# EryiXie/PlaneRecNet

Measured on AMD Instinct MI355X. Metric: img/s fwd+bwd @480×640 ResNet101-DCN, 1/2/4/8 MI355X + roofline %, higher is better.
Workload: dtype f32 (tensors and accumulation fp32; plain GEMMs and the tap-walked 4x4/s2, 1x1/s2 and sub-pixel convolutions >= 300 tiles: 2xfp16-piece split MFMA, fp32 accumulate; fp32-only rate in fp32_only_run)

## Files before the change

### planerecnet_amd/csrc/prn_wgrad16.hip

```cpp
#include "prn_common.h"

namespace {

typedef __attribute__((ext_vector_type(8))) _Float16 h8_t;
typedef __attribute__((ext_vector_type(2))) _Float16 h2_t;
typedef __attribute__((ext_vector_type(2))) float f2_t;
typedef __attribute__((ext_vector_type(16))) float f16x_t;

constexpr unsigned W16_OOB = 0x80000000u;
constexpr int W16_PLANE = 128 * 32;
constexpr int W16_BUF = 4 * W16_PLANE;

struct Wg16Args {
  const float* dy; const float* x; float* out;
  int M, C, HW, B;
  int N;
  int tilesM, tilesC, splits, chunks;
  long long zdy, zx;
  long long zout;
  int nz;
  int wide;
  int ngroup;
  const float* gx[PRN_WGRAD_GROUP_MAX];
  const float* gdy[PRN_WGRAD_GROUP_MAX];
};

__device__ __forceinline__ const float* w16_kernarg_ptr(size_t member_offset, int i) {
  typedef __attribute__((address_space(4))) const uint64_t* kptr;
  kptr base = (kptr)__builtin_amdgcn_kernarg_segment_ptr();
  return reinterpret_cast<const float*>(base[member_offset / 8 + i]);
}

__device__ __forceinline__ float quad_max(float v) {
  const int a = __builtin_amdgcn_mov_dpp(__float_as_int(v), 0xB1, 0xF, 0xF, true);
  v = fmaxf(v, __int_as_float(a));
  const int b = __builtin_amdgcn_mov_dpp(__float_as_int(v), 0x4E, 0xF, 0xF, true);
  return fmaxf(v, __int_as_float(b));
}

template <int NP>
__global__ __launch_bounds__(256) __attribute__((amdgpu_waves_per_eu(3, 3))) void wgrad16_kernel(const Wg16Args a) {
  __shared__ __attribute__((aligned(16))) unsigned char pieces[2 * W16_BUF];
  __shared__ int rowexp[2][256];
  __shared__ int scratch[4][64];
  const int t = threadIdx.x, lane = t & 63, wave = __builtin_amdgcn_readfirstlane(t >> 6);
  const int tiles = a.tilesM * a.tilesC;
  const int lid = prn_xcd_remap(blockIdx.x, tiles * a.splits * a.nz);
  const int tile = lid % tiles, rest = lid / tiles;
  const int tm = tile % a.tilesM, tc = tile / a.tilesM;
  const int sp = rest % a.splits, z = rest / a.splits;
  const int q0 = (int)((long long)a.chunks * sp / a.splits), q1 = (int)((long long)a.chunks * (sp + 1) / a.splits);
  const int HW = a.HW;
  const float* dyz = a.ngroup > 0 ? w16_kernarg_ptr(offsetof(Wg16Args, gdy), z) : a.dy + (long long)z * a.zdy;
  const float* xz = a.ngroup > 0 ? w16_kernarg_ptr(offsetof(Wg16Args, gx), z) : a.x + (long long)z * a.zx;
  const __amdgpu_buffer_rsrc_t ars = __builtin_amdgcn_make_buffer_rsrc(const_cast<float*>(dyz), 0, a.B * a.M * HW * 4, 0x00020000);
  const __amdgpu_buffer_rsrc_t brs = __builtin_amdgcn_make_buffer_rsrc(const_cast<float*>(xz), 0, a.B * a.C * HW * 4, 0x00020000);

  const int quarter = t & 3, rsub = t >> 2;
  unsigned rowoff[4];
  int erun[4];
  unsigned wroff[4];
#pragma unroll
  for (int k = 0; k < 4; ++k) {
    const int rl = rsub + 64 * (k & 1);
    const int row = (k < 2 ? tm : tc) * 128 + rl;
    const bool ok = row < (k < 2 ? a.M : a.C);
    rowoff[k] = ok ? (unsigned)(row * HW * 4) : W16_OOB;
    erun[k] = -200;
    wroff[k] = (unsigned)((k < 2 ? 0 : 2 * W16_PLANE) + rl * 32 + (((quarter >> 1) ^ ((rl >> 2) & 1)) * 16) + (quarter & 1) * 8);
  }
  const unsigned imgA = (unsigned)(a.M * HW * 4), imgB = (unsigned)(a.C * HW * 4);
  int cb, cp;
  {
    const long long n = (long long)q0 * 16 + quarter * 4;
    cb = (int)(n / HW); cp = (int)(n - (long long)cb * HW);
  }
  float4 ld0[4], ld1[4];
  auto load_chunk = [&](float4 (&ld)[4]) {
    const unsigned past = (unsigned)((a.B - 1 - cb) >> 31) << 31;
    const unsigned pa = ((unsigned)cb * imgA + (unsigned)cp * 4u) | past, pb = ((unsigned)cb * imgB + (unsigned)cp * 4u) | past;
#pragma unroll
    for (int k = 0; k < 4; ++k)
      ld[k] = __builtin_bit_cast(float4, __builtin_amdgcn_raw_buffer_load_b128(k < 2 ? ars : brs, (int)((k < 2 ? pa : pb) + (rowoff[k] & 0x7fffffffu)) | (int)(rowoff[k] & 0x80000000u), 0, 0));
    cp += 16;
    const int wrap = (HW - 1 - cp) >> 31;
    cp -= HW & wrap; cb -= wrap;
  };
  auto cut_chunk = [&](const float4 (&ld)[4], int buf) {
    unsigned char* pb = pieces + buf * W16_BUF;
#pragma unroll
    for (int k = 0; k < 4; ++k) {
      const float4 v = ld[k];
      const float mx = quad_max(fmaxf(fmaxf(fabsf(v.x), fabsf(v.y)), fmaxf(fabsf(v.z), fabsf(v.w))));
      int ec = mx > 0.f ? __builtin_amdgcn_frexp_expf(mx) : -200;
      ec = ec < -100 ? (mx > 0.f ? -100 : -200) : ec;
      if (ec > erun[k] + 3) erun[k] = ec;
      const float s = __builtin_amdgcn_ldexpf(1.0f, 11 - (erun[k] < -100 ? -100 : erun[k]));
      const f2_t s2 = {s, s};
      const f2_t x0 = f2_t{v.x, v.y} * s2, x1 = f2_t{v.z, v.w} * s2;
      const h2_t h0 = __builtin_convertvector(x0, h2_t), h1 = __builtin_convertvector(x1, h2_t);
      const f2_t r0 = x0 - __builtin_convertvector(h0, f2_t), r1 = x1 - __builtin_convertvector(h1, f2_t);
      const h2_t l0 = __builtin_convertvector(r0, h2_t), l1 = __builtin_convertvector(r1, h2_t);
      uint2 hh, ll;
      hh.x = __builtin_bit_cast(unsigned, h0); hh.y = __builtin_bit_cast(unsigned, h1);
      ll.x = __builtin_bit_cast(unsigned, l0); ll.y = __builtin_bit_cast(unsigned, l1);
      *reinterpret_cast<uint2*>(pb + wroff[k]) = hh;
      *reinterpret_cast<uint2*>(pb + wroff[k] + W16_PLANE) = ll;
      if (quarter == 0) rowexp[buf][rsub + 64 * k] = erun[k];
    }
  };

  const int wm = wave >> 1, wn = wave & 1, r = lane & 31, g = lane >> 5;
  f16x_t acc[2][2];
#pragma unroll
  for (int i = 0; i < 2; ++i)
#pragma unroll
    for (int j = 0; j < 2; ++j)
#pragma unroll
      for (int e = 0; e < 16; ++e) acc[i][j][e] = 0.f;
  int prevA = -200, prevB = -200;
  auto mma_chunk = [&](int buf) {
    const int newA = rowexp[buf][wm * 64 + lane], newB = rowexp[buf][128 + wn * 64 + lane];
    const int dA = prevA - newA, dB = prevB - newB;
    prevA = newA; prevB = newB;
    if (__builtin_amdgcn_ballot_w64((dA | dB) != 0) != 0ull) {
      scratch[wave][lane] = dA;
      __builtin_amdgcn_wave_barrier();
#pragma unroll
      for (int j = 0; j < 2; ++j) {
        const int db = __shfl(dB, j * 32 + r, 64);
#pragma unroll
        for (int i = 0; i < 2; ++i)
#pragma unroll
          for (int e = 0; e < 16; ++e) {
            const int da = scratch[wave][i * 32 + (e >> 2) * 8 + g * 4 + (e & 3)];
            acc[i][j][e] = __builtin_amdgcn_ldexpf(acc[i][j][e], da + db);
          }
      }
      __builtin_amdgcn_wave_barrier();
    }
    const unsigned char* pb = pieces + buf * W16_BUF;
    h8_t ah[2], al[2], bh[2], bl[2];
#pragma unroll
    for (int u = 0; u < 2; ++u) {
      const int ra = wm * 64 + u * 32 + r, rb = wn * 64 + u * 32 + r;
      const unsigned oa = (unsigned)(ra * 32 + ((g ^ ((ra >> 2) & 1)) * 16)), ob = (unsigned)(2 * W16_PLANE + rb * 32 + ((g ^ ((rb >> 2) & 1)) * 16));
      ah[u] = *reinterpret_cast<const h8_t*>(pb + oa); al[u] = *reinterpret_cast<const h8_t*>(pb + oa + W16_PLANE);
      bh[u] = *reinterpret_cast<const h8_t*>(pb + ob); bl[u] = *reinterpret_cast<const h8_t*>(pb + ob + W16_PLANE);
    }
#pragma unroll
    for (int i = 0; i < 2; ++i)
#pragma unroll
      for (int j = 0; j < 2; ++j) {
        f16x_t c = acc[i][j];
        if (NP >= 4) c = __builtin_amdgcn_mfma_f32_32x32x16_f16(al[i], bl[j], c, 0, 0, 0);
        c = __builtin_amdgcn_mfma_f32_32x32x16_f16(al[i], bh[j], c, 0, 0, 0);
        c = __builtin_amdgcn_mfma_f32_32x32x16_f16(ah[i], bl[j], c, 0, 0, 0);
        c = __builtin_amdgcn_mfma_f32_32x32x16_f16(ah[i], bh[j], c, 0, 0, 0);
        acc[i][j] = c;
      }
  };

  const int nq = q1 - q0;
  if (nq > 0) {
    load_chunk(ld0);
    load_chunk(ld1);
    cut_chunk(ld0, 0);
    load_chunk(ld0);
    __syncthreads();
    int i = 0;
    for (; i + 1 < nq; i += 2) {
      cut_chunk(ld1, 1);
      load_chunk(ld1);
      __builtin_amdgcn_sched_barrier(0);
      mma_chunk(0);
      __syncthreads();
      cut_chunk(ld0, 0);
      load_chunk(ld0);
      __builtin_amdgcn_sched_barrier(0);
      mma_chunk(1);
      __syncthreads();
    }
    if (i < nq) mma_chunk(0);
  }

  scratch[wave][lane] = prevA;
  __builtin_amdgcn_wave_barrier();
  float* ob = a.out + ((long long)sp * a.nz + z) * a.zout;
  if (a.wide) {
    __syncthreads();
    float* cw = reinterpret_cast<float*>(pieces) + wave * (32 * 36);
    const int crow = lane >> 3, ccol = (lane & 7) * 4;
#pragma unroll
    for (int j = 0; j < 2; ++j) {
      const int eb = __shfl(prevB, j * 32 + r, 64);
      const int col4 = tc * 128 + wn * 64 + j * 32 + ccol;
#pragma unroll
      for (int i = 0; i < 2; ++i) {
#pragma unroll
        for (int e = 0; e < 16; ++e) {
          const int ro = (e >> 2) * 8 + g * 4 + (e & 3);
          const int ea = scratch[wave][i * 32 + ro];
          cw[ro * 36 + r] = (ea <= -200 || eb <= -200) ? 0.f : __builtin_amdgcn_ldexpf(acc[i][j][e], ea + eb - 22);
        }
        __builtin_amdgcn_wave_barrier();
#pragma unroll
        for (int q = 0; q < 4; ++q) {
          const int rl = crow + 8 * q, row = tm * 128 + wm * 64 + i * 32 + rl;
          const float4 v = *reinterpret_cast<const float4*>(&cw[rl * 36 + ccol]);
          if (row < a.M && col4 < a.C) *reinterpret_cast<float4*>(ob + (long long)row * a.C + col4) = v;
        }
        __builtin_amdgcn_wave_barrier();
      }
    }
    return;
  }
#pragma unroll
  for (int j = 0; j < 2; ++j) {
    const int col = tc * 128 + wn * 64 + j * 32 + r;
    const int eb = __shfl(prevB, j * 32 + r, 64);
    if (col >= a.C) continue;
#pragma unroll
    for (int i = 0; i < 2; ++i)
#pragma unroll
      for (int e = 0; e < 16; ++e) {
        const int rl = i * 32 + (e >> 2) * 8 + g * 4 + (e & 3), row = tm * 128 + wm * 64 + rl;
        const int ea = scratch[wave][rl];
        if (row < a.M) ob[(long long)row * a.C + col] = (ea <= -200 || eb <= -200) ? 0.f : __builtin_amdgcn_ldexpf(acc[i][j][e], ea + eb - 22);
      }
  }
}

}

int prn_wgrad16_plan(int M, int C, int64_t N, int HW, int nz, const prn_gemm_opts* o) {
  if (o == nullptr || o->wgrad_split == PRN_SPLIT_OFF) return 0;
  if (M <= 0 || C <= 0 || N <= 0 || nz <= 0 || nz >= 65536 || (HW & 3) != 0 || HW < 16 || N % HW != 0) return 0;
  if ((int64_t)M * N >= (1LL << 29) || (int64_t)C * N >= (1LL << 29)) return 0;
  const int64_t tiles = (int64_t)cdiv(M, 128) * cdiv(C, 128) * nz;
  const int chunks = cdiv(N, 16);
  if (o->wgrad_split != PRN_SPLIT_ALWAYS) {
    if ((int64_t)cdiv(M, 128) * 128 * 4 > (int64_t)M * 5 || (int64_t)cdiv(C, 128) * 128 * 4 > (int64_t)C * 5) return 0;
    if (2.0 * M * C * (double)N * nz < 0.25e9 * (double)o->split_min_gflop) return 0;
  }
  const int target = o->wgrad_wgs > 0 ? o->wgrad_wgs : 768;
  int64_t s = tiles >= target ? 1 : target / tiles;
  const int smax = chunks / 8 > 0 ? chunks / 8 : 1;
  if (s > smax) s = smax;
  if (s > 256) s = 256;
  s = prn_quantise_splits(tiles, (int)s);
  return s < 1 ? 1 : (int)s;
}

int prn_wgrad16_launch(const float* dy, const float* x, const float* const* gdy, const float* const* gx, int ngroup, float* out, int M, int C, int B, int HW, int nz,
                       int64_t zdy, int64_t zx, int splits, const prn_gemm_opts* o, hipStream_t st) {
  PRN_REQUIRE(out && splits >= 1 && (ngroup > 0 ? (gdy && gx && ngroup <= PRN_WGRAD_GROUP_MAX) : (dy && x)), "prn_wgrad16: bad arguments");
  Wg16Args a;
  a.dy = dy; a.x = x; a.out = out; a.M = M; a.C = C; a.HW = HW; a.B = B; a.N = B * HW;
  a.tilesM = cdiv(M, 128); a.tilesC = cdiv(C, 128); a.splits = splits; a.chunks = cdiv((int64_t)B * HW, 16);
  a.zdy = zdy; a.zx = zx; a.zout = (long long)M * C; a.nz = ngroup > 0 ? ngroup : nz; a.ngroup = ngroup;
  for (int i = 0; i < PRN_WGRAD_GROUP_MAX; ++i) {
    a.gx[i] = ngroup > 0 ? gx[i < ngroup ? i : 0] : nullptr; a.gdy[i] = ngroup > 0 ? gdy[i < ngroup ? i : 0] : nullptr;
    if (ngroup > 0) {
      PRN_REQUIRE(a.gx[i] && a.gdy[i] && (reinterpret_cast<uintptr_t>(a.gx[i]) & 15) == 0 && (reinterpret_cast<uintptr_t>(a.gdy[i]) & 15) == 0, "prn_wgrad16: null / unaligned tensor in the group");
    }
  }
  a.wide = (C & 3) == 0 && (reinterpret_cast<uintptr_t>(out) & 15) == 0;
  const dim3 grid((unsigned)(a.tilesM * a.tilesC * splits * a.nz)), block(256);
  if (o && o->split_products >= 4) hipLaunchKernelGGL(wgrad16_kernel<4>, grid, block, 0, st, a);
  else hipLaunchKernelGGL(wgrad16_kernel<3>, grid, block, 0, st, a);
  PRN_CHECK_LAUNCH("prn_wgrad16");
  return 0;
}
```

Measured before the change: 194.9.

## Interleave fp16 split conversion of next chunk with MFMAs in wgrad16

Adds a CUT variant of the split-fp16 weight-gradient kernel, enabled by default. It scans the next chunk's row maxima up front using integer bit comparisons and a cached scale/threshold, so exponents are recomputed only when a row's magnitude grows. The hi/lo split conversion and LDS stores are cut into parts and placed between the MFMA instructions of the current chunk, so VALU conversion work overlaps matrix work instead of running serially before it. It also uses v_max3 and fma_mix inline asm. The cost is higher register pressure, more sched_barrier constraints, and some risk that the read-before-write ordering on the alternate LDS buffer is wrong.

```diff
diff --git a/planerecnet_amd/csrc/prn_wgrad16.hip b/planerecnet_amd/csrc/prn_wgrad16.hip
--- a/planerecnet_amd/csrc/prn_wgrad16.hip
+++ b/planerecnet_amd/csrc/prn_wgrad16.hip
@@ -38,7 +38,21 @@
   return fmaxf(v, __int_as_float(b));
 }
 
-template <int NP>
+__device__ __forceinline__ unsigned quad_max_bits(unsigned v) {
+  const unsigned a = (unsigned)__builtin_amdgcn_update_dpp(0, (int)v, 0xB1, 0xF, 0xF, true);
+  v = v > a ? v : a;
+  const unsigned b = (unsigned)__builtin_amdgcn_update_dpp(0, (int)v, 0x4E, 0xF, 0xF, true);
+  return v > b ? v : b;
+}
+
+__device__ __forceinline__ unsigned absmax4_bits(const float4 v) {
+  float m;
+  asm("v_max3_f32 %0, |%1|, |%2|, |%3|" : "=v"(m) : "v"(v.x), "v"(v.y), "v"(v.z));
+  const unsigned mb = __float_as_uint(m), wb = __float_as_uint(v.w) & 0x7fffffffu;
+  return mb > wb ? mb : wb;
+}
+
+template <int NP, int CUT>
 __global__ __launch_bounds__(256) __attribute__((amdgpu_waves_per_eu(3, 3))) void wgrad16_kernel(const Wg16Args a) {
   __shared__ __attribute__((aligned(16))) unsigned char pieces[2 * W16_BUF];
   __shared__ int rowexp[2][256];
@@ -59,6 +73,8 @@
   const int quarter = t & 3, rsub = t >> 2;
   unsigned rowoff[4];
   int erun[4];
+  float scl[4];
+  int thr[4];
   unsigned wroff[4];
 #pragma unroll
   for (int k = 0; k < 4; ++k) {
@@ -66,7 +82,7 @@
     const int row = (k < 2 ? tm : tc) * 128 + rl;
     const bool ok = row < (k < 2 ? a.M : a.C);
     rowoff[k] = ok ? (unsigned)(row * HW * 4) : W16_OOB;
-    erun[k] = -200;
+    erun[k] = -200; scl[k] = 0x1p+111f; thr[k] = 1;
     wroff[k] = (unsigned)((k < 2 ? 0 : 2 * W16_PLANE) + rl * 32 + (((quarter >> 1) ^ ((rl >> 2) & 1)) * 16) + (quarter & 1) * 8);
   }
   const unsigned imgA = (unsigned)(a.M * HW * 4), imgB = (unsigned)(a.C * HW * 4);
@@ -78,10 +94,14 @@
   float4 ld0[4], ld1[4];
   auto load_chunk = [&](float4 (&ld)[4]) {
     const unsigned past = (unsigned)((a.B - 1 - cb) >> 31) << 31;
-    const unsigned pa = ((unsigned)cb * imgA + (unsigned)cp * 4u) | past, pb = ((unsigned)cb * imgB + (unsigned)cp * 4u) | past;
+    const unsigned pa0 = (unsigned)cb * imgA + (unsigned)cp * 4u, pb0 = (unsigned)cb * imgB + (unsigned)cp * 4u;
+    const unsigned pa = pa0 | past, pb = pb0 | past;
 #pragma unroll
     for (int k = 0; k < 4; ++k)
-      ld[k] = __builtin_bit_cast(float4, __builtin_amdgcn_raw_buffer_load_b128(k < 2 ? ars : brs, (int)((k < 2 ? pa : pb) + (rowoff[k] & 0x7fffffffu)) | (int)(rowoff[k] & 0x80000000u), 0, 0));
+      if (CUT)
+        ld[k] = __builtin_bit_cast(float4, __builtin_amdgcn_raw_buffer_load_b128(k < 2 ? ars : brs, (int)(((k < 2 ? pa0 : pb0) + rowoff[k]) | past), 0, 0));
+      else
+        ld[k] = __builtin_bit_cast(float4, __builtin_amdgcn_raw_buffer_load_b128(k < 2 ? ars : brs, (int)((k < 2 ? pa : pb) + (rowoff[k] & 0x7fffffffu)) | (int)(rowoff[k] & 0x80000000u), 0, 0));
     cp += 16;
     const int wrap = (HW - 1 - cp) >> 31;
     cp -= HW & wrap; cb -= wrap;
@@ -110,6 +130,55 @@
     }
   };
 
+  auto cut_scan = [&](const float4 (&ld)[4], int buf) {
+    int epub = rowexp[buf ^ 1][rsub + 64 * quarter];
+    unsigned mx[4];
+    bool grow = false;
+#pragma unroll
+    for (int k = 0; k < 4; ++k) {
+      mx[k] = quad_max_bits(absmax4_bits(ld[k]));
+      grow |= (int)mx[k] >= thr[k];
+    }
+    if (__builtin_amdgcn_ballot_w64(grow) != 0ull) {
+#pragma unroll
+      for (int k = 0; k < 4; ++k) {
+        int e = rowexp[buf ^ 1][rsub + 64 * k];
+        const float m = __uint_as_float(mx[k]);
+        int ec = m > 0.f ? __builtin_amdgcn_frexp_expf(m) : -200;
+        ec = ec < -100 ? (m > 0.f ? -100 : -200) : ec;
+        if (ec > e + 3) e = ec;
+        scl[k] = __builtin_amdgcn_ldexpf(1.0f, 11 - (e < -100 ? -100 : e));
+        thr[k] = e < -100 ? 1 : (e + 130 > 255 ? 255 : e + 130) << 23;
+        epub = quarter == k ? e : epub;
+      }
+    }
+    rowexp[buf][rsub + 64 * quarter] = epub;
+  };
+  float cx[4]; h2_t ch[2];
+  auto cut_part = [&](const float4 (&ld)[4], int buf, int k, int part) {
+    if (part == 0) {
+      const f2_t s2 = {scl[k], scl[k]};
+      const f2_t x0 = f2_t{ld[k].x, ld[k].y} * s2, x1 = f2_t{ld[k].z, ld[k].w} * s2;
+      cx[0] = x0[0]; cx[1] = x0[1]; cx[2] = x1[0]; cx[3] = x1[1];
+      ch[0] = __builtin_convertvector(x0, h2_t); ch[1] = __builtin_convertvector(x1, h2_t);
+    } else if (part == 1) {
+#pragma unroll
+      for (int e = 0; e < 2; ++e) {
+        const unsigned h = __builtin_bit_cast(unsigned, ch[e]);
+        asm("v_fma_mix_f32 %0, %1, -1.0, %2 op_sel:[0,0,0] op_sel_hi:[1,0,0]" : "=v"(cx[2 * e]) : "v"(h), "v"(cx[2 * e]));
+        asm("v_fma_mix_f32 %0, %1, -1.0, %2 op_sel:[1,0,0] op_sel_hi:[1,0,0]" : "=v"(cx[2 * e + 1]) : "v"(h), "v"(cx[2 * e + 1]));
+      }
+    } else {
+      unsigned char* pb = pieces + buf * W16_BUF;
+      const h2_t l0 = __builtin_convertvector(f2_t{cx[0], cx[1]}, h2_t), l1 = __builtin_convertvector(f2_t{cx[2], cx[3]}, h2_t);
+      uint2 hh, ll;
+      hh.x = __builtin_bit_cast(unsigned, ch[0]); hh.y = __builtin_bit_cast(unsigned, ch[1]);
+      ll.x = __builtin_bit_cast(unsigned, l0); ll.y = __builtin_bit_cast(unsigned, l1);
+      *reinterpret_cast<uint2*>(pb + wroff[k]) = hh;
+      *reinterpret_cast<uint2*>(pb + wroff[k] + W16_PLANE) = ll;
+    }
+  };
+
   const int wm = wave >> 1, wn = wave & 1, r = lane & 31, g = lane >> 5;
   f16x_t acc[2][2];
 #pragma unroll
@@ -119,44 +188,76 @@
 #pragma unroll
       for (int e = 0; e < 16; ++e) acc[i][j][e] = 0.f;
   int prevA = -200, prevB = -200;
-  auto mma_chunk = [&](int buf) {
+  auto mma_rescale = [&](int buf) {
     const int newA = rowexp[buf][wm * 64 + lane], newB = rowexp[buf][128 + wn * 64 + lane];
     const int dA = prevA - newA, dB = prevB - newB;
     prevA = newA; prevB = newB;
     if (__builtin_amdgcn_ballot_w64((dA | dB) != 0) != 0ull) {
       scratch[wave][lane] = dA;
       __builtin_amdgcn_wave_barrier();
-#pragma unroll
-      for (int j = 0; j < 2; ++j) {
-        const int db = __shfl(dB, j * 32 + r, 64);
-#pragma unroll
-        for (int i = 0; i < 2; ++i)
+      if (CUT) {
+        const int db0 = __shfl(dB, r, 64), db1 = __shfl(dB, 32 + r, 64);
+#pragma unroll
+        for (int i = 0; i < 2; ++i) {
 #pragma unroll
           for (int e = 0; e < 16; ++e) {
             const int da = scratch[wave][i * 32 + (e >> 2) * 8 + g * 4 + (e & 3)];
-            acc[i][j][e] = __builtin_amdgcn_ldexpf(acc[i][j][e], da + db);
+            acc[i][0][e] = __builtin_amdgcn_ldexpf(acc[i][0][e], da + db0);
+            acc[i][1][e] = __builtin_amdgcn_ldexpf(acc[i][1][e], da + db1);
           }
+          __builtin_amdgcn_sched_barrier(0);
+        }
+      } else {
+#pragma unroll
+        for (int j = 0; j < 2; ++j) {
+          const int db = __shfl(dB, j * 32 + r, 64);
+#pragma unroll
+          for (int i = 0; i < 2; ++i)
+#pragma unroll
+            for (int e = 0; e < 16; ++e) {
+              const int da = scratch[wave][i * 32 + (e >> 2) * 8 + g * 4 + (e & 3)];
+              acc[i][j][e] = __builtin_amdgcn_ldexpf(acc[i][j][e], da + db);
+            }
+        }
       }
       __builtin_amdgcn_wave_barrier();
     }
+  };
+  auto mma_chunk = [&](int buf, const float4 (*ld)[4]) {
+    mma_rescale(buf);
     const unsigned char* pb = pieces + buf * W16_BUF;
+    const bool cut = CUT && ld != nullptr;
     h8_t ah[2], al[2], bh[2], bl[2];
-#pragma unroll
-    for (int u = 0; u < 2; ++u) {
-      const int ra = wm * 64 + u * 32 + r, rb = wn * 64 + u * 32 + r;
-      const unsigned oa = (unsigned)(ra * 32 + ((g ^ ((ra >> 2) & 1)) * 16)), ob = (unsigned)(2 * W16_PLANE + rb * 32 + ((g ^ ((rb >> 2) & 1)) * 16));
+    auto read_a = [&](int u) {
+      const int ra = wm * 64 + u * 32 + r;
+      const unsigned oa = (unsigned)(ra * 32 + ((g ^ ((ra >> 2) & 1)) * 16));
       ah[u] = *reinterpret_cast<const h8_t*>(pb + oa); al[u] = *reinterpret_cast<const h8_t*>(pb + oa + W16_PLANE);
+    };
+    auto read_b = [&](int u) {
+      const int rb = wn * 64 + u * 32 + r;
+      const unsigned ob = (unsigned)(2 * W16_PLANE + rb * 32 + ((g ^ ((rb >> 2) & 1)) * 16));
       bh[u] = *reinterpret_cast<const h8_t*>(pb + ob); bl[u] = *reinterpret_cast<const h8_t*>(pb + ob + W16_PLANE);
-    }
+    };
+    read_a(0); read_b(0);
+    if (!cut) read_a(1);
+    read_b(1);
 #pragma unroll
     for (int i = 0; i < 2; ++i)
 #pragma unroll
       for (int j = 0; j < 2; ++j) {
         f16x_t c = acc[i][j];
+        const int k = i * 2 + j;
         if (NP >= 4) c = __builtin_amdgcn_mfma_f32_32x32x16_f16(al[i], bl[j], c, 0, 0, 0);
+        if (cut) { cut_part(*ld, buf ^ 1, k, 0); __builtin_amdgcn_sched_barrier(0); }
         c = __builtin_amdgcn_mfma_f32_32x32x16_f16(al[i], bh[j], c, 0, 0, 0);
+        if (cut) { __builtin_amdgcn_sched_barrier(0); cut_part(*ld, buf ^ 1, k, 1); __builtin_amdgcn_sched_barrier(0); }
         c = __builtin_amdgcn_mfma_f32_32x32x16_f16(ah[i], bl[j], c, 0, 0, 0);
+        if (cut) { __builtin_amdgcn_sched_barrier(0); cut_part(*ld, buf ^ 1, k, 2); __builtin_amdgcn_sched_barrier(0); }
         c = __builtin_amdgcn_mfma_f32_32x32x16_f16(ah[i], bh[j], c, 0, 0, 0);
+        if (cut) {
+          __builtin_amdgcn_sched_barrier(0);
+          if (k == 0) { read_a(1); __builtin_amdgcn_sched_barrier(0); }
+        }
         acc[i][j] = c;
       }
   };
@@ -165,23 +266,44 @@
   if (nq > 0) {
     load_chunk(ld0);
     load_chunk(ld1);
-    cut_chunk(ld0, 0);
+    if (CUT) {
+      rowexp[1][rsub + 64 * quarter] = -200;
+      cut_scan(ld0, 0);
+#pragma unroll
+      for (int k = 0; k < 4; ++k)
+        for (int part = 0; part < 3; ++part) cut_part(ld0, 0, k, part);
+    } else {
+      cut_chunk(ld0, 0);
+    }
     load_chunk(ld0);
     __syncthreads();
     int i = 0;
-    for (; i + 1 < nq; i += 2) {
-      cut_chunk(ld1, 1);
-      load_chunk(ld1);
-      __builtin_amdgcn_sched_barrier(0);
-      mma_chunk(0);
-      __syncthreads();
-      cut_chunk(ld0, 0);
-      load_chunk(ld0);
-      __builtin_amdgcn_sched_barrier(0);
-      mma_chunk(1);
-      __syncthreads();
-    }
-    if (i < nq) mma_chunk(0);
+    if (CUT) {
+      for (; i + 1 < nq; i += 2) {
+        cut_scan(ld1, 1);
+        mma_chunk(0, &ld1);
+        load_chunk(ld1);
+        __syncthreads();
+        cut_scan(ld0, 0);
+        mma_chunk(1, &ld0);
+        load_chunk(ld0);
+        __syncthreads();
+      }
+    } else {
+      for (; i + 1 < nq; i += 2) {
+        cut_chunk(ld1, 1);
+        load_chunk(ld1);
+        __builtin_amdgcn_sched_barrier(0);
+        mma_chunk(0, nullptr);
+        __syncthreads();
+        cut_chunk(ld0, 0);
+        load_chunk(ld0);
+        __builtin_amdgcn_sched_barrier(0);
+        mma_chunk(1, nullptr);
+        __syncthreads();
+      }
+    }
+    if (i < nq) mma_chunk(0, nullptr);
   }
 
   scratch[wave][lane] = prevA;
@@ -267,8 +389,16 @@
   }
   a.wide = (C & 3) == 0 && (reinterpret_cast<uintptr_t>(out) & 15) == 0;
   const dim3 grid((unsigned)(a.tilesM * a.tilesC * splits * a.nz)), block(256);
-  if (o && o->split_products >= 4) hipLaunchKernelGGL(wgrad16_kernel<4>, grid, block, 0, st, a);
-  else hipLaunchKernelGGL(wgrad16_kernel<3>, grid, block, 0, st, a);
+  const char* cutenv = getenv("PRN_WGRAD16_CUT");
+  const bool cut = !(cutenv && atoi(cutenv) == 0);
+  const bool np4 = o && o->split_products >= 4;
+  if (cut) {
+    if (np4) hipLaunchKernelGGL((wgrad16_kernel<4, 1>), grid, block, 0, st, a);
+    else hipLaunchKernelGGL((wgrad16_kernel<3, 1>), grid, block, 0, st, a);
+  } else {
+    if (np4) hipLaunchKernelGGL((wgrad16_kernel<4, 0>), grid, block, 0, st, a);
+    else hipLaunchKernelGGL((wgrad16_kernel<3, 0>), grid, block, 0, st, a);
+  }
   PRN_CHECK_LAUNCH("prn_wgrad16");
   return 0;
 }
```

New measurement: 195.2, median of 5. About the same (+0.1%).
